# HDSRL/SRB-CBF-NMPC

Hardware: AMD Instinct MI355X
Metric: NMPC solves/sec (whole node) + p99 solve latency, N-agent batch horizon=10 (higher is better)
Workload: dtype f64; 1 GPU; 1024 agents/GPU, horizon 10, 3 static + 8-nearest inter-agent CBF, fp64; agents_per_gpu=1024, agents_total=1024, horizon=10, contacts=2, K_obs=3, K_nbr=8, parallelism=agents sharded x1, n_obs=5120, nbr_rows=1024

## Files before the change

srb-cbf-nmpc_amd/csrc/srb_gram.h:

```cpp
#pragma once
#include <hip/hip_runtime.h>
#include <stdint.h>
#include <type_traits>
#include <utility>
#include "srb_kernel_params.h"
#include "srb_wave.h"

struct TermLayout {
    int N, C, n, nz, E4;
    __device__ __forceinline__ int zr(int v) const { return v < 4 * N ? v : v + E4; }
};

struct ObsFold {
    const double *OJ;
    double *FO;
    int rO, N, K, NOP;
    uint64_t mask;
    int rU, C, n;
};

template <int NZL, bool GRAM, bool RHS>
__device__ __forceinline__ void ul_add(const double *R, const double *W, const double *CF, const ObsFold &F, double *H,
                                       double *g, int nz, int tid0, int step)
{
    constexpr int LDR = NZL + 1, LDH = NZL + 1;
    const int c1 = F.C - 1, np = F.N * c1 * c1, rl = F.rU + 2 * F.N, rs = F.rU + F.n - 1 - 4 * F.N;
    if (GRAM) {
        for (int e = tid0; e <= np; e += step) {
            if (e == np) { H[0] = H[0] + W[rs]; continue; }
            const int j = e / (c1 * c1), rem = e - j * c1 * c1, a = 1 + j * c1 + rem / c1, b = 1 + j * c1 + rem % c1;
            double wv[6], ra[6], rb[6];
#pragma unroll
            for (int u = 0; u < 6; u++) {
                const bool in = u < 2 + F.C;
                const int r = (u < 2) ? F.rU + 2 * j + u : rl + F.C * j + (in ? u - 2 : 0);
                wv[u] = in ? W[r] : 0.0; ra[u] = in ? R[r * LDR + a] : 0.0; rb[u] = in ? R[r * LDR + b] : 0.0;
            }
            const double h0 = H[a * LDH + b];
            __builtin_amdgcn_sched_barrier(0);
            double v = 0.0;
#pragma unroll
            for (int u = 0; u < 6; u++) {
                if (u >= 2 + F.C) break;
                v = fma(wv[u] * ra[u], rb[u], v);
            }
            H[a * LDH + b] = h0 + v;
        }
    }
    if (RHS) {
        for (int a = tid0; a < nz; a += step) {
            if (a == 0) { g[0] += CF[rs]; continue; }
            const int j = (a - 1) / c1;
            double cv[6], ra[6];
#pragma unroll
            for (int u = 0; u < 6; u++) {
                const bool in = u < 2 + F.C;
                const int r = (u < 2) ? F.rU + 2 * j + u : rl + F.C * j + (in ? u - 2 : 0);
                cv[u] = in ? CF[r] : 0.0; ra[u] = in ? R[r * LDR + a] : 0.0;
            }
            const double g0 = g[a];
            __builtin_amdgcn_sched_barrier(0);
            double v = 0.0;
#pragma unroll
            for (int u = 0; u < 6; u++) {
                if (u >= 2 + F.C) break;
                v = fma(cv[u], ra[u], v);
            }
            g[a] = g0 + v;
        }
    }
}

template <int NZL>
struct UlLane {
    double wv[6], ra[6], rb[6], cv[6], sw, sc;
    int q;
    bool he, ge, hs;
    template <bool GRAM, bool RHS>
    __device__ __forceinline__ void load(const double *R, const double *W, const double *CF, const ObsFold &F, int nz, int lane)
    {
        constexpr int LDR = NZL + 1;
        const int li = lane & 15, kq = lane >> 4;
        const int c1 = F.C - 1, rl = F.rU + 2 * F.N, rs = F.rU + F.n - 1 - 4 * F.N;
        const bool col = li >= 1 && li < nz;
        const int j = col ? (li - 1) / c1 : 0, a0 = 1 + j * c1, off = (kq - a0) & 3;
        he = GRAM && col && off < c1;
        ge = RHS && col && kq == 0;
        hs = lane == 0;
        const int a = he ? a0 + off : 1, b = col ? li : 1;
        q = a >> 2;
#pragma unroll
        for (int u = 0; u < 6; u++) {
            const bool in = u < 2 + F.C;
            const int r = (u < 2) ? F.rU + 2 * j + u : rl + F.C * j + (in ? u - 2 : 0);
            if (GRAM) { wv[u] = W[r]; ra[u] = R[r * LDR + a]; }
            rb[u] = R[r * LDR + b];
            if (RHS) cv[u] = CF[r];
        }
        if (GRAM) sw = W[rs];
        if (RHS) sc = CF[rs];
    }
    template <bool GRAM, bool RHS>
    __device__ __forceinline__ void sums(const ObsFold &F, double &vh, double &vg) const
    {
        vh = 0.0; vg = 0.0;
#pragma unroll
        for (int u = 0; u < 6; u++) {
            if (u >= 2 + F.C) break;
            if (GRAM) vh = fma(wv[u] * ra[u], rb[u], vh);
            if (RHS) vg = fma(cv[u], rb[u], vg);
        }
    }
};

template <bool GRAM>
__device__ __forceinline__ void obs_fold(const double *W, const double *CF, const ObsFold &F, int tid, int NTH)
{
    for (int k = tid; k < F.N; k += NTH) {
        double s00 = 0.0, s01 = 0.0, s02 = 0.0, s11 = 0.0, s12 = 0.0, s22 = 0.0, c0 = 0.0, c1 = 0.0, c2 = 0.0;
        for (int j0 = 0; j0 < F.K; j0 += 8) {
            double cfv[8], jxv[8], jyv[8], wv[8];
#pragma unroll
            for (int u = 0; u < 8; u++) {
                const bool in = j0 + u < F.K;
                const int o = k * F.K + (in ? j0 + u : 0);
                cfv[u] = in ? CF[F.rO + o] : 0.0; jxv[u] = in ? F.OJ[2 * o] : 0.0; jyv[u] = in ? F.OJ[2 * o + 1] : 0.0;
                wv[u] = (GRAM && in) ? W[F.rO + o] : 0.0;
            }
#pragma unroll
            for (int u = 0; u < 8; u++) {
                if (j0 + u >= F.K) break;
                const double cf = cfv[u], jx = jxv[u], jy = jyv[u];
                c0 = fma(cf, jx, c0); c1 = fma(cf, jy, c1); c2 -= cf;
                if (GRAM) {
                    const double w = wv[u], wx = w * jx, wy = w * jy;
                    s00 = fma(wx, jx, s00); s01 = fma(wx, jy, s01); s02 -= wx; s11 = fma(wy, jy, s11); s12 -= wy; s22 += w;
                }
            }
        }
        double *f = F.FO + 9 * k;
        if (GRAM) { f[0] = s00; f[1] = s01; f[2] = s02; f[3] = s11; f[4] = s12; f[5] = s22; }
        f[6] = c0; f[7] = c1; f[8] = c2;
    }
}

__device__ __forceinline__ int term_maxcol(int t, int N, int C, int n, int rC, int NE, int rU)
{
    const int c1 = C - 1;
    if (t < rC) return (t / 4 + 1) * c1;
    if (t < rC + NE) return ((t - rC) / 2 + 2) * c1;
    if (t < rU) return 0;
    const int v = 4 * N + (t - rU);
    if (v < 6 * N) return ((v - 4 * N) / 2 + 1) * c1;
    if (v < n - 1) return ((v - 6 * N) / C + 1) * c1;
    return 0;
}

template <int NZM>
__device__ __forceinline__ uint64_t full_batches(int rO, int N, int C, int n, int rC, int NE, int rU, int lane)
// ... 418 lines not shown
            g[tid] = v;
        }
        __syncthreads();
        ul_add<NZL, true, RHS>(R, W, CF, F, H, g, nz, tid, 64 * NW);
    }
}

template <int NZL, int NW>
__device__ __forceinline__ void rhs_only(const double *R, const double *CF, int cnt, const ObsFold &F, int nko, double *g,
                                         int nz, int tid, double *part, uint64_t bmask)
{
    constexpr int NZM = ((NZL + 15) / 16) * 16;
    constexpr int NTC = NZM / 16;
    const int lane = tid & 63, wv = tid >> 6;
    const int li = lane & 15, kq = lane >> 4;
    constexpr bool FOLD = !SRB_OBS_STORED(NZL);
    if (FOLD && nko > 0) {
        obs_fold<false>(nullptr, CF, F, tid, 64 * NW);
        srb_sync<NW>();
    }
    double ps[2][NTC];
    constexpr bool ULF = NZM == 16 && NW == 1;
    UlLane<NZL> ul;
    double ulh = 0.0, ulg = 0.0;
#pragma unroll
    for (int t = 0; t < NTC; t++) { ps[0][t] = 0.0; ps[1][t] = 0.0; }
    auto chunk32 = [&](int t0, auto fullc) {
        constexpr int NB = decltype(fullc)::value ? NTC : 1;
        double a[8][NTC], c[8];
#pragma unroll
        for (int u = 0; u < 8; u++) {
            const int r = t0 + 4 * u + kq;
            c[u] = CF[r];
#pragma unroll
            for (int tc = 0; tc < NB; tc++) a[u][tc] = term_elem<NZL>(R, r, 16 * tc + li);
        }
        __builtin_amdgcn_sched_barrier(0);
#pragma unroll
        for (int u = 0; u < 8; u++)
#pragma unroll
            for (int tc = 0; tc < NB; tc++) ps[u & 1][tc] = fma(c[u], a[u][tc], ps[u & 1][tc]);
    };
    auto schunk16 = [&](int t0, auto fullc) {
        constexpr int NB = decltype(fullc)::value ? NTC : 1;
        double a[4][NTC], c[4];
#pragma unroll
        for (int u = 0; u < 4; u++) {
            const int r = t0 + 4 * u + kq;
            c[u] = CF[r];
#pragma unroll
            for (int tc = 0; tc < NB; tc++) a[u][tc] = term_elem<NZL>(R, r, 16 * tc + li);
        }
        __builtin_amdgcn_sched_barrier(0);
#pragma unroll
        for (int u = 0; u < 4; u++)
#pragma unroll
            for (int tc = 0; tc < NB; tc++) ps[u & 1][tc] = fma(c[u], a[u][tc], ps[u & 1][tc]);
    };
    auto ochunk16 = [&](int t0, auto fullc) {
        constexpr int NB = decltype(fullc)::value ? NTC : 1;
        double a[4][NTC], c[4];
#pragma unroll
        for (int u = 0; u < 4; u++) {
            const int t = t0 + 4 * u + kq, k = t / 3, uu = t - 3 * k;
            c[u] = F.FO[9 * min(k, F.N) + 6 + uu];
#pragma unroll
            for (int tc = 0; tc < NB; tc++) {
                double zx, zy;
                a[u][tc] = obs_term_a<NZL>(R, F, t, 16 * tc + li, zx, zy);
            }
        }
        __builtin_amdgcn_sched_barrier(0);
#pragma unroll
        for (int u = 0; u < 4; u++)
#pragma unroll
            for (int tc = 0; tc < NB; tc++) ps[u & 1][tc] = fma(c[u], a[u][tc], ps[u & 1][tc]);
    };
    auto range = [&](int tb, int te, bool st) {
        int t0 = tb;
#pragma clang loop unroll(disable)
        for (; t0 + 32 <= te; t0 += 32) {
            if (NZM == 16 || st || batch_full(bmask, t0) || batch_full(bmask, t0 + 16))
                chunk32(t0, std::integral_constant<bool, true>{});
            else
                chunk32(t0, std::integral_constant<bool, false>{});
        }
#pragma clang loop unroll(disable)
        for (; t0 < te; t0 += 4) {
            const int r = t0 + kq;
            const double cc = CF[r];
#pragma unroll
            for (int tc = 0; tc < NTC; tc++) ps[0][tc] = fma(cc, term_elem<NZL>(R, r, 16 * tc + li), ps[0][tc]);
        }
    };
    if constexpr (ULF) ul.template load<false, true>(R, nullptr, CF, F, nz, lane);
    {
        constexpr bool ILV = NZM == 32 && NW > 1;
        const int chunk = cnt / NW, tb = wv * chunk;
        if constexpr (ILV) {
#pragma clang loop unroll(disable)
            for (int t0 = 16 * wv; t0 < cnt; t0 += 16 * NW) {
                if (batch_full(bmask, t0)) schunk16(t0, std::integral_constant<bool, true>{});
                else schunk16(t0, std::integral_constant<bool, false>{});
            }
        } else {
            range(tb, tb + chunk, false);
        }
        if (!FOLD && nko > 0) {
            const int och = nko / NW, ob = F.rO + wv * och;
            range(ob, ob + och, true);
        }
        if (FOLD && nko > 0) {
            const int och = F.NOP / NW, ob = ILV ? 16 * wv : wv * och, oe = ILV ? F.NOP : ob + och, os = ILV ? 16 * NW : 16;
#pragma clang loop unroll(disable)
            for (int o0 = ob; o0 < oe; o0 += os) {
                if (NZM == 16 || batch_full(F.mask, o0)) ochunk16(o0, std::integral_constant<bool, true>{});
                else ochunk16(o0, std::integral_constant<bool, false>{});
            }
        }
    }
    if constexpr (ULF) ul.template sums<false, true>(F, ulh, ulg);
    double sv[NTC];
#pragma unroll
    for (int tc = 0; tc < NTC; tc++) sv[tc] = chunk_sum16(ps[0][tc] + ps[1][tc]);
    if constexpr (NW <= 2) {
#pragma unroll
        for (int ph = 0; ph < NW; ph++) {
            if (ph > 0) __syncthreads();
            if (wv == ph) {
#pragma unroll
                for (int tc = 0; tc < NTC; tc++)
                    if (kq == 0 && 16 * tc + li < nz) {
                        if constexpr (ULF) g[li] = ul.ge ? sv[0] + ulg : ul.hs ? sv[0] + ul.sc : sv[0];
                        else g[16 * tc + li] = ph ? g[16 * tc + li] + sv[tc] : sv[tc];
                    }
                if (ph == NW - 1 && !ULF) ul_add<NZL, false, true>(R, nullptr, CF, F, nullptr, g, nz, lane, 64);
            }
        }
    } else {
#pragma unroll
        for (int tc = 0; tc < NTC; tc++)
            if (kq == 0) part[wv * NZM + 16 * tc + li] = sv[tc];
        __syncthreads();
        if (tid < nz) {
            double v = 0.0;
#pragma unroll
            for (int w2 = 0; w2 < NW; w2++) v += part[w2 * NZM + tid];
            g[tid] = v;
        }
        __syncthreads();
        ul_add<NZL, false, true>(R, nullptr, CF, F, nullptr, g, nz, tid, 64 * NW);
    }
}
```

srb-cbf-nmpc_amd/csrc/srb_kernels.hip:

```cpp
#include <hip/hip_runtime.h>
#include <stdint.h>
#include <type_traits>
#include "srb_kernel_params.h"
#include "srb_kernel_decls.h"

#define WAVE 64
#include "srb_wave.h"
#include "srb_gj.h"
#include "srb_solve.h"
#include "srb_gram.h"
#define SYNC() srb_sync<NW>()

#ifdef SRB_STAMPS
#define SRB_NSTAMP 64
__device__ unsigned long long srb_stamp_buf[SRB_NSTAMP];
#define STAMP_DECL unsigned long long st_t0 = 0; int st_off = 0
#define STAMP_BEGIN() do { __builtin_amdgcn_sched_barrier(0); st_t0 = __builtin_amdgcn_s_memtime(); __builtin_amdgcn_sched_barrier(0); } while (0)
#define STAMP_END(slot) do { __builtin_amdgcn_sched_barrier(0); const unsigned long long _t = __builtin_amdgcn_s_memtime(); \
    __builtin_amdgcn_sched_barrier(0); if (threadIdx.x == 0 && stamp_lds) atomicAdd(&stamp_lds[st_off + (slot)], _t - st_t0); st_t0 = _t; } while (0)
#define STAMP_STAGE(s) (st_off = 32 * (s))
#define STAMP_FLUSH(agent) do { SYNC(); if ((agent) == 0 && threadIdx.x < 64) atomicAdd(&srb_stamp_buf[threadIdx.x], stamp_lds[threadIdx.x]); } while (0)
#else
#define STAMP_DECL do {} while (0)
#define STAMP_BEGIN() do {} while (0)
// ... 137 lines not shown
#define SK_KIND(q, t) (TK::compiled ? TK::kind(q, t) : kind_of(q))
#define SK_EQ(t, kd, k) (TK::compiled ? TK::eq(t, kd, k) : (kd) == (k))
#define SK_M(q, t, r) (TK::compiled ? TK::m(q, t, r) : (q).m[r])
#define SK_TWO(t) (!TK::compiled || TK::two(t))
#define SK_ON(t) (TK::compiled && TK::on(t))
#define SK_COM(t) (!TK::compiled || TK::com(t))

template <class TK>
__device__ __forceinline__ double slot_fx(const Slot &q, int t, double x0, double x1, double s_var)
{
    const int k = SK_KIND(q, t);
    const double dx = x0 - q.a0, dy = x1 - q.a1;
    return SK_EQ(t, k, K_OBS) ? -(dx * dx + dy * dy) - s_var : SK_EQ(t, k, K_COP) ? x0 - x1 : x0;
}
template <class TK>
__device__ __forceinline__ double slot_f(const Slot &q, int t, const double *xs, double s_var)
{
    return slot_fx<TK>(q, t, xs[q.i0], xs[q.i1], s_var);
}



__device__ __forceinline__ double zo_sum(const double *zo, int k, int K)
{
    const double *z = zo + k * K;
    double s = 0.0;
    for (int j0 = 0; j0 < K; j0 += 16) {
        double v[16];
#pragma unroll
        for (int u = 0; u < 16; u++) v[u] = (j0 + u < K) ? z[j0 + u] : 0.0;
#pragma unroll
        for (int u = 0; u < 16; u++) s += v[u];
    }
    return s;
}

__device__ __forceinline__ void slot_init(Slot &q, int sl, const SrbKParams &prm, const TermLayout &TL, const double *ref,
                                          int sE, int sV, int sO, int S, int rC, int rO, int K, int TT)
{
    const int N = prm.N, n = prm.n;
    q.kind = K_NONE; q.i0 = q.i1 = 0; q.r = 0; q.h[0] = q.h[1] = 0.0; q.a0 = q.a1 = 0.0; q.rx = 0.0; q.jd = 0.0;
    q.m[0] = q.m[1] = 0.0; q.wr = TT;
    if (sl < SRB_SLOT_END(K_VAR, sE, sV, sO, S)) {
        const int v = sl;
        const bool isX = v < 4 * N, isU = !isX && v < 6 * N, isL = !isX && !isU && v < n - 1;
        q.kind = K_VAR; q.i0 = q.i1 = v; q.r = TL.zr(v);
        q.a0 = isX ? ((v >= 4 * (N - 1)) ? prm.Pw : prm.Qw) : isU ? prm.Rw : isL ? 0.0 : prm.Sw;
        q.a1 = isX ? -q.a0 * ref[v] : 0.0;
        q.h[0] = isL ? 1.0 : prm.box; q.h[1] = isL ? 0.0 : prm.box;
    } else if (sl < SRB_SLOT_END(K_COP, sE, sV, sO, S)) {
        const int e = sl - sE, i = e >> 1, d = e & 1;
        q.kind = K_COP; q.i0 = 4 * i + 2 * d; q.i1 = 4 * N + 2 * (i + 1) + d; q.r = rC + e;
        q.h[0] = q.h[1] = prm.fr;
    } else if (sl < SRB_SLOT_END(K_VEL, sE, sV, sO, S)) {
        const int tt = sl - sV, comp = (tt < N) ? 1 : 3, k = tt % N;
        q.kind = K_VEL; q.i0 = q.i1 = 4 * k + comp; q.r = 4 * k + comp;
        q.h[0] = q.h[1] = prm.vsat;
    } else if (sl < SRB_SLOT_END(K_OBS, sE, sV, sO, S)) {
        const int o = sl - sO, k = o / K;
        q.kind = K_OBS; q.i0 = 4 * k; q.i1 = 4 * k + 2; q.r = rO + o;
    }
#pragma unroll
    for (int r = 0; r < 2; r++) { q.s[r] = q.z[r] = 1.0; q.iz[r] = q.is[r] = 1.0; q.dz[r] = q.ds[r] = q.dsT[r] = q.r3[r] = 0.0; }
}

template <class TK>
__device__ __forceinline__ void slot_stage(Slot &q, int t, int n, bool nl, int TT)
{
    const bool lin = (SK_ISP(q, t, K_VAR) && (SK_ON(t) || q.i0 < n - 1)) || SK_ISP(q, t, K_COP);
    q.m[0] = (lin || (nl && (SK_ISP(q, t, K_VEL) || SK_ISP(q, t, K_OBS)))) ? 1.0 : 0.0;
    q.m[1] = (lin || (nl && SK_ISP(q, t, K_VEL))) ? 1.0 : 0.0;
    q.wr = (SK_ISP(q, t, K_VAR) || SK_ISP(q, t, K_COP) || SK_ISP(q, t, K_OBS)) ? q.r : TT;
}

#define SRB_SLOT_LCK(q, sl) do { \
    LCK((q).wr <= TT, 2); \
    LCK((q).kind == K_NONE || ((q).i0 >= 0 && (q).i0 < n && (q).i1 >= 0 && (q).i1 < n), 3); \
    LCK(!((q).kind == K_VAR || (q).kind == K_COP || (q).kind == K_VEL || ((q).kind == K_OBS && SRB_OBS_STORED(NZL))) || \
        ((q).r >= 0 && (q).r < RROWS), 1); \
    LCK((q).kind != K_OBS || ((sl) - sO >= 0 && (sl) - sO < NK && (q).r - rO == (sl) - sO), 5); \
} while (0)

__device__ __forceinline__ double var_weight(const SrbKParams &prm, int v)
{
    const int N = prm.N;
    return v < 4 * N ? ((v >= 4 * (N - 1)) ? prm.Pw : prm.Qw) : v < 6 * N ? prm.Rw : v < prm.n - 1 ? 0.0 : prm.Sw;
}

template <int NZL, int TS, int NW, class TK>
__device__ __forceinline__ void polish_rows(Slot (&Q)[TS], int nts, const double *xs, double *OJ, double *zo, int n,
                                            int rO, double *R, int nz)
{
    const double s_var = xs[n - 1];
#pragma unroll
    for (int t = 0; t < TS; t++)
        if (t < nts) {
            Slot &q = Q[t];
            q.jd = slot_f<TK>(q, t, xs, s_var);
            if (SK_IS(q, t, K_OBS)) {
                const int o = q.r - rO;
                obs_relin<NZL>(R, OJ, rO, o, q.i0, q.i1, -2.0 * (xs[q.i0] - q.a0), -2.0 * (xs[q.i1] - q.a1));
                zo[o] = q.ds[0] * q.dz[0];
            }
        }
}

__device__ __forceinline__ double lip_eq_res(const SrbKParams &prm, const double *x0, const double *xs, const double *foot,
                                             int N, int C, int tid, int NTH)
{
    double r = 0.0;
#if defined(SRB_DIAG_FLAT_EQRES)
#ifndef SRB_DIAG_BUILD
#error "SRB_DIAG_FLAT_EQRES is a diagnostic-build option"
#endif
    for (int k = tid; k < N; k += NTH) {
        const double *xp = k ? xs + 4 * (k - 1) : x0;
        const double p0 = xp[0], p1 = xp[1], p2 = xp[2], p3 = xp[3];
#else
    const double g0x = x0[0], g1x = x0[1], g2x = x0[2], g3x = x0[3];
    for (int k = tid; k < N; k += NTH) {
        const int kp = k ? k - 1 : 0;
        const double p0 = k ? xs[4 * kp] : g0x, p1 = k ? xs[4 * kp + 1] : g1x;
        const double p2 = k ? xs[4 * kp + 2] : g2x, p3 = k ? xs[4 * kp + 3] : g3x;
#endif
        const double u0 = xs[4 * N + 2 * k], u1 = xs[4 * N + 2 * k + 1];
#pragma unroll
        for (int d = 0; d < 4; d++) {
            const double v = prm.Ad[4 * d] * p0 + prm.Ad[4 * d + 1] * p1 + prm.Ad[4 * d + 2] * p2 +
                             prm.Ad[4 * d + 3] * p3 + prm.Bd[2 * d] * u0 + prm.Bd[2 * d + 1] * u1;
            r = fmax(r, fabs(xs[4 * k + d] - v));
        }
        double g0 = 0.0, g1 = 0.0, sl = 0.0;
#pragma unroll
        for (int j = 0; j < 4; j++)
            if (j < C) {
                const double lam = xs[6 * N + C * k + j];
                g0 = fma(foot[(2 * k) * C + j], lam, g0); g1 = fma(foot[(2 * k + 1) * C + j], lam, g1); sl += lam;
            }
        r = fmax(r, fmax(fabs(u0 - g0), fmax(fabs(u1 - g1), fabs(sl - 1.0))));
    }
    return r;
}

template <int NZL, int TS, int NW, int NZE, class TK>
__device__ __forceinline__ double polish_stationary(Slot (&Q)[TS], int nts, const SrbKParams &prm, const double *xs,
                                                  const double *ref, double *CF, double *R, double *OJ, double *zo, int rO,
                                                  int cnt, const ObsFold &OF, int nko, double *vg, double *vy, double *vr,
                                                  double *vd, const double (&Mi)[NZL], const double *H0, int nz, int tid,
                                                  double *part, uint64_t bmask, double *red, int N, int n, int TT, int srow)
{
    SYNC();
    polish_rows<NZL, TS, NW, TK>(Q, nts, xs, OJ, zo, n, rO, R, nz);
    SYNC();
#pragma unroll
    for (int t = 0; t < TS; t++)
        if (t < nts) {
            const Slot &q = Q[t];
            const double zj = SK_TWO(t) ? q.ds[0] * q.dz[0] - q.ds[1] * q.dz[1] : q.ds[0] * q.dz[0];
            const int kd = SK_KIND(q, t);
            if (SK_EQ(t, kd, K_VAR)) {
                const int v = q.i0;
                const double a0 = var_weight(prm, v), gf = fma(a0, xs[v], (v < 4 * N) ? -a0 * ref[v] : 0.0);
                CF[q.wr] = gf + zj;
            } else if (SK_EQ(t, kd, K_COP) || SK_EQ(t, kd, K_OBS)) {
                CF[q.wr] = zj;
            }
        }
    if (NW > 1) SYNC();
#pragma unroll
    for (int t = 0; t < TS; t++)
        if (t < nts && SK_IS(Q[t], t, K_VEL))
            __hip_atomic_fetch_add(&CF[Q[t].r], Q[t].ds[0] * Q[t].dz[0] - Q[t].ds[1] * Q[t].dz[1], __ATOMIC_RELAXED,
                                   __HIP_MEMORY_SCOPE_WORKGROUP);
    SYNC();
    rhs_only<NZL, NW>(R, CF, cnt, OF, nko, vg, nz, tid, part, bmask);
    SYNC();
    double dxs[NZL];
    la_solve<NZL, NW, NZE>(Mi, H0, H0, 0.0, vg, vy, vr, vd, dxs, nz, tid & 63);
    double dm = 0.0;
#pragma unroll
    for (int j = 0; j < NZL; j++) dm = fmax(dm, fabs(dxs[j]));
    constexpr int LDR = NZL + 1;
    double zmin = 1e300, zmax = 1.0;
#pragma unroll
    for (int t = 0; t < TS; t++)
        if (t < nts && (Q[t].ds[0] != 0.0 || (SK_TWO(t) && Q[t].ds[1] != 0.0))) {
            const Slot &q = Q[t];
            const double jd = -((!SRB_OBS_STORED(NZL) && SK_IS(q, t, K_OBS))
                ? fma(OJ[2 * (q.r - rO)], row_dot<NZL, NZE>(R + q.i0 * LDR, dxs),
                      fma(OJ[2 * (q.r - rO) + 1], row_dot<NZL, NZE>(R + q.i1 * LDR, dxs), -row_dot<NZL, NZE>(R + srow * LDR, dxs)))
                : row_dot<NZL, NZE>(R + q.r * LDR, dxs));
#pragma unroll
            for (int r = 0; r < 2; r++)
                if ((SK_TWO(t) || r == 0) && q.ds[r] != 0.0) {
                    const double zn = fma(prm.polish_rho, q.r3[r] + (r ? -jd : jd), q.dz[r]);
                    zmin = fmin(zmin, zn); zmax = fmax(zmax, fabs(zn));
                }
        }
    double rv[2] = {-zmin, zmax};
    wred_x<2, 3u, NW>(rv, red + 5 * 8 * NW, tid);
    return (-rv[0] >= -(prm.polish_rho * SRB_POLISH_PTOL + 1e-9 * rv[1])) ? dm : 1e300;
}

#define SRB_AGENT_LAYOUT \
    constexpr int NZM = ((NZL + 15) / 16) * 16; \
    constexpr int LDR = NZL + 1, LDH = NZL + 1; \
    constexpr int NTH = 64 * NW; \
    constexpr int NZE = (NC > 0 && CC > 0) ? NC * (CC - 1) + 1 : NZL;    \
     \
    constexpr bool GVEC = SRB_GRAM_FORM != SRB_GRAM_MFMA && srb_shape_compiled(NC, CC, KC) && NW == 1 && NZL <= 12 && \
                          SRB_OBS_STORED(NZL) && CC > 1 && NZE <= NZL; \
    using GSH = GramShape<GVEC ? NC : 0, GVEC ? CC : 0, GVEC ? KC : 0>; \
    const int tid = threadIdx.x, lane = tid & 63, wv = tid >> 6; \
     \
    const int N = NC > 0 ? NC : prm.N, C = CC > 0 ? CC : prm.C, K = KC > 0 ? KC : prm.K_obs + prm.K_nbr; \
    const int n = (NC > 0 && CC > 0) ? (6 + CC) * NC + 1 : prm.n, nz = (NC > 0 && CC > 0) ? NC * (CC - 1) + 1 : prm.nz; \
    const int NK = N * K, NE = 2 * (N - 1); \
    const int n4 = rnd4(n), NK4 = rnd4(NK), UL4 = rnd4(n - 4 * N); \
    const int E4 = (4 * N + NE + 16 * NW - 1) / (16 * NW) * (16 * NW) - 4 * N;    \
     \
     \
    const int rC = 4 * N, rU = rC + E4, rO = (rU + UL4 + 16 * NW - 1) / (16 * NW) * (16 * NW); \
    const int NKP = (NK + 16 * NW - 1) / (16 * NW) * (16 * NW), TT = rO + NKP; \
    const TermLayout TL{N, C, n, nz, E4}; \
    const uint64_t bmask = full_batches<NZM>(rO, N, C, n, rC, NE, rU, lane);    \
    const int NOP = (3 * N + 16 * NW - 1) / (16 * NW) * (16 * NW);    \
    const int sE = n, sV = n + NE, sO = sV + 2 * N, S = sO + NK; \
    const double tol = prm.tol, th = tol / sqrt(3.0); \
    STAMP_DECL; \
     \
    double *p = lds; \
    double *R = p; p += (SRB_OBS_STORED(NZL) ? TT : rO) * LDR;    \
    double *W = p; p += TT + 1;                    \
    double *CF = p; p += TT + 1;                   \
    double *OJ = p; p += SRB_OBS_STORED(NZL) ? 0 : 2 * NKP;        \
    double *FO = p; p += SRB_OBS_STORED(NZL) ? 0 : 9 * (N + 1);    \
    const ObsFold OF{OJ, FO, rO, N, K, NOP, full_obs_batches<NZM>(N, C, NOP, lane), rU, C, n}; \
    double *H0 = p; p += NZL * LDH;                \
    double *ZZ = p; p += NZL * LDH;                \
    double *vg = p; p += NZM; double *vy = p; p += NZM; double *vr = p; p += NZM; double *vd = p; p += NZM; \
    double *xs = p; p += n4; \
    double *xb = p; p += n4;                       \
    double *dxv = xb; \
    double *xsv = p; p += n4;                      \
    double *xprev = p; p += n4;                    \
    double *ref = p; p += 4 * N; \
    double *foot = p; p += 2 * C * N; \
    double *obs = SRB_OBS_IN_ZZ(NZL, NK) ? ZZ : p; p += SRB_OBS_IN_ZZ(NZL, NK) ? 0 : 2 * NK + 2;    \
    double *eps = p; p += K + 1; \
    double *zo = p; p += NK4;                      \
    int *sel = (int *)p; p += (K + 1); \
    double *red = p; p += (NW > 1) ? 8 * SRB_RED_SITES * NW : 0;    \
    double *part = p; p += (NW > 2) ? NW * ((NZM == 16) ? 1 : 3) * 256 + NW * NZM : 0;    \
    float *zpl = (float *)p; p += SRB_FUSED_POLISH_OK(NZL) ? rnd4(S) : 0;    \
    const int RROWS = SRB_OBS_STORED(NZL) ? TT : rO;    \
    LCK_INIT(); \
    LCK((int)(p - lds) <= srb_lds_doubles(prm, NZL, NW), 0); \
    LCK(rU <= RROWS && (!SRB_OBS_STORED(NZL) || rO + NKP <= TT), 4); \
    (void)RROWS; \
    do {} while (0)

#define SRB_AGENT_SETUP \
    const double *x0 = x0g + 4 * (size_t)agent; \
    for (int i = tid; i < 4 * N; i += NTH) ref[i] = refg[(size_t)agent * 4 * N + i]; \
    for (int i = tid; i < 2 * C * N; i += NTH) foot[i] = footg[(size_t)agent * 2 * C * N + i]; \
    if (prm.use_nlp && tid < K) sel[tid] = sel_g[(size_t)agent * K + tid]; \
    for (int i = tid; i < (int)(xs - R) + 2 * n4; i += NTH) R[i] = 0.0; \
    for (int i = tid; i < NK4; i += NTH) zo[i] = 0.0; \
    SYNC(); \
    STAMP_END(23);                  \
    if (prm.use_nlp) { SRB_AGENT_OBSTACLES; } \
    STAMP_END(24);                  \
     \
    if (tid == 0) { \
        double X[4] = {x0[0], x0[1], x0[2], x0[3]}; \
        for (int k = 0; k < N; k++) { \
            const double u0 = foot[(k * 2 + 0) * C + C - 1], u1 = foot[(k * 2 + 1) * C + C - 1]; \
            double Xn[4]; \
            for (int d = 0; d < 4; d++) \
                Xn[d] = prm.Ad[d * 4] * X[0] + prm.Ad[d * 4 + 1] * X[1] + prm.Ad[d * 4 + 2] * X[2] + prm.Ad[d * 4 + 3] * X[3] + \
                        prm.Bd[d * 2] * u0 + prm.Bd[d * 2 + 1] * u1; \
            for (int d = 0; d < 4; d++) { X[d] = Xn[d]; xb[4 * k + d] = Xn[d]; } \
            xb[4 * N + 2 * k] = u0; xb[4 * N + 2 * k + 1] = u1; \
            for (int j = 0; j < C; j++) xb[6 * N + C * k + j] = (j == C - 1) ? 1.0 : 0.0; \
        } \
        xb[n - 1] = 0.0; \
    } \
    for (int cg = tid; cg < nz - 1; cg += NTH) {    \
        const int j = cg / (C - 1), t = cg % (C - 1), col = cg + 1; \
        double lam[4]; \
        const int is_null = lambda_basis(foot + j * 2 * C, C, t, lam); \
        double g0 = 0.0, g1 = 0.0; \
        if (!is_null) \
            _Pragma("unroll") for (int i = 0; i < 4; i++) \
                if (i < C) { g0 += foot[(j * 2 + 0) * C + i] * lam[i]; g1 += foot[(j * 2 + 1) * C + i] * lam[i]; } \
        _Pragma("unroll") for (int i = 0; i < 4; i++) if (i < C) R[TL.zr(6 * N + C * j + i) * LDR + col] = lam[i]; \
        R[TL.zr(4 * N + 2 * j) * LDR + col] = g0; \
        R[TL.zr(4 * N + 2 * j + 1) * LDR + col] = g1; \
        double v[4]; \
        for (int d = 0; d < 4; d++) v[d] = prm.Bd[d * 2] * g0 + prm.Bd[d * 2 + 1] * g1; \
        for (int k = j; k < N; k++) { \
            for (int d = 0; d < 4; d++) R[(4 * k + d) * LDR + col] = v[d]; \
            double tt[4]; \
            for (int d = 0; d < 4; d++) tt[d] = prm.Ad[d * 4] * v[0] + prm.Ad[d * 4 + 1] * v[1] + prm.Ad[d * 4 + 2] * v[2] + prm.Ad[d * 4 + 3] * v[3]; \
            for (int d = 0; d < 4; d++) v[d] = tt[d]; \
        } \
    } \
    if (tid == 0) R[TL.zr(n - 1) * LDR] = 1.0; \
    SYNC(); \
    STAMP_END(25);                  \
     \
    if (tid < NE) { \
        const int i = tid >> 1, d = tid & 1, pp = 4 * i + 2 * d, uu = 4 * N + 2 * (i + 1) + d; \
        for (int a = 0; a < NZL; a++) Rt[tid * LDR + a] = R[pp * LDR + a] - R[TL.zr(uu) * LDR + a]; \
    } \
    for (int v = tid; v < n; v += NTH) xs[v] = xb[v]; \
    do {} while (0)

#define SRB_AGENT_OBSTACLES \
     \
    { \
        double ox_[TS], oy_[TS]; \
        _Pragma("unroll") for (int t = 0; t < TS; t++) { \
            const int e = tid + NTH * t; \
            ox_[t] = oy_[t] = 0.0; \
            if (e < NK) { \
                const int k = e / K, j = e - k * K; \
                const bool st = j < prm.K_obs; \
                const int bi = sel[j]; \
                const double tt = st ? 0.0 : prm.Ts * (k + 1); \
                const size_t bj = (bi >= 0) ? bi : 0; \
                if (nbr_plan) {    \
                     \
                    const double *srcp = st ? obstacles + 2 * bj : nbr_plan + 2 * (bj * (size_t)N + k); \
                    ox_[t] = (bi >= 0) ? srcp[0] : x0[0] + 1000.0; \
                    oy_[t] = (bi >= 0) ? srcp[1] : x0[2]; \
                } else { \
                    const double *srcp = st ? obstacles + 2 * bj : nbr_state + 4 * bj; \
                     \
                    ox_[t] = (bi >= 0) ? srcp[0] + (st ? 0.0 : srcp[2] * tt) : x0[0] + 1000.0; \
                    oy_[t] = (bi >= 0) ? srcp[1] + (st ? 0.0 : srcp[3] * tt) : x0[2]; \
                } \
                if (MV && obs_vel) {    \
                     \
                     \
                     \
                    _Pragma("clang fp contract(off)") \
                    if (st && bi >= 0) { \
                        const double tk = prm.Ts * (k + 1); \
                        ox_[t] = obstacles[2 * bj] + obs_vel[2 * bj] * tk; \
                        oy_[t] = obstacles[2 * bj + 1] + obs_vel[2 * bj + 1] * tk; \
                    } \
                } \
            } \
        } \
        _Pragma("unroll") for (int t = 0; t < TS; t++) { \
            const int e = tid + NTH * t; \
            if (e < NK) { obs[2 * e] = ox_[t]; obs[2 * e + 1] = oy_[t]; } \
        } \
        if (tid < K) eps[tid] = (tid < prm.K_obs) ? prm.eps_obs : prm.eps_nbr; \
         \
         \
         \
        if (MV && obs_eps) { if (tid < prm.K_obs && sel[tid] >= 0) eps[tid] = obs_eps[sel[tid]]; } \
         \
// ... 521 lines not shown
```

srb-cbf-nmpc_amd/csrc/srb_stage_body.h:

```cpp
        const double tolS = (!nl && prm.use_nlp && prm.qp_warm_tol > 0.0) ? prm.qp_warm_tol : tol, thS = tolS / sqrt(3.0);
        STAMP_STAGE(stage);
        const int nts = ((nl ? S : sV) + NTH - 1) / NTH;
        const int mrows = nl ? (4 * (N - 1) + 12 * N + 2 * C * N + NK + 4 * N) : (4 * (N - 1) + 12 * N + 2 * C * N);
        const int cnt = rU, nko = nl ? NKP : 0;
        STAMP_BEGIN();
#pragma unroll
        for (int t = 0; t < TS; t++) {
            Slot &q = Q[t];
            const bool lin = (SK_ISP(q, t, K_VAR) && (SK_ON(t) || q.i0 < n - 1)) || SK_ISP(q, t, K_COP);
            q.m[0] = (lin || (nl && (SK_ISP(q, t, K_VEL) || SK_ISP(q, t, K_OBS)))) ? 1.0 : 0.0;
            q.m[1] = (lin || (nl && SK_ISP(q, t, K_VEL))) ? 1.0 : 0.0;
            q.wr = (SK_ISP(q, t, K_VAR) || SK_ISP(q, t, K_COP) || SK_ISP(q, t, K_OBS)) ? q.r : TT;
        }
        if (!nl) {
#pragma unroll
            for (int t = 0; t < TS; t++)
                if (SK_TWO(t) && t < nts) {
                    Slot &q = Q[t];
                    const double f = slot_f<TK>(q, t, xs, 0.0);
                    const double w0 = SK_M(q, t, 0) * (q.h[0] - f), w1 = SK_M(q, t, 1) * (q.h[1] + f);
                    const bool var = SK_ISP(q, t, K_VAR);
                    const double wgt = (var ? q.a0 : 0.0) + SK_M(q, t, 0) + SK_M(q, t, 1);
                    const double cfv = (var ? -q.a1 - q.a0 * f : 0.0) + (w0 - w1);
                    if (SK_ISP(q, t, K_VAR) || SK_ISP(q, t, K_COP)) { W[q.r] = wgt; CF[q.r] = cfv; }
// ... 92 lines not shown
#pragma unroll
            for (int t = 0; t < TS; t++)
                if (t < nts) {
                    Slot &q = Q[t];
                    const double f = q.jd;
                    q.s[0] = (SK_M(q, t, 0) != 0.0) ? q.h[0] - f + ssh : 1.0;
                    if (SK_TWO(t)) q.s[1] = (SK_M(q, t, 1) != 0.0) ? q.h[1] + f + ssh : 1.0;
                    q.z[0] = SRB_NLP_Z0 * rcp_d(fmax(q.s[0], 1.0));
                    if (SK_TWO(t)) q.z[1] = SRB_NLP_Z0 * rcp_d(fmax(q.s[1], 1.0));
                    if (SK_ISP(q, t, K_OBS)) {
                        const int o = q.r - rO;
                        obs_relin<NZL>(R, OJ, rO, o, q.i0, q.i1, -2.0 * (xs[q.i0] - q.a0), -2.0 * (xs[q.i1] - q.a1));
                    }
                    const double jz = SK_TWO(t) ? SK_M(q, t, 0) * q.z[0] - SK_M(q, t, 1) * q.z[1] : q.m[0] * q.z[0];
                    if (SK_ISP(q, t, K_VAR)) { W[q.r] = 1.0; CF[q.r] = fma(q.a0, f, q.a1) + jz; }
                    else if (SK_ISP(q, t, K_COP)) { W[q.r] = 0.0; CF[q.r] = jz; }
                    else if (SK_ISP(q, t, K_OBS)) { W[q.r] = 0.0; CF[q.r] = q.z[0]; }
                }
            if (NW > 1) SYNC();
#pragma unroll
            for (int t = 0; t < TS; t++)
                if (t < nts && SK_ISP(Q[t], t, K_VEL))
                    __hip_atomic_fetch_add(&CF[Q[t].r], Q[t].m[0] * Q[t].z[0] - Q[t].m[1] * Q[t].z[1], __ATOMIC_RELAXED,
                                           __HIP_MEMORY_SCOPE_WORKGROUP);
            SYNC();
            if constexpr (GVEC) gram_rhs_vec<NZL, true, GSH, SRB_GRAM_FORM>(R, W, CF, OF, nko, ZZ, vg, nz, lane);
            else gram_rhs<NZL, true, NW>(R, W, CF, cnt, OF, nko, ZZ, vg, nz, tid, part, bmask);
            SYNC();
            gj_load<NZL, NZE>(Mi, ZZ, ZZ, 0.0, nz, lane);
            gj_factor<NZL, NZE>(Mi, nz, lane, 0);
            la_solve<NZL, NW, NZE>(Mi, ZZ, ZZ, 0.0, vg, vy, vr, vd, dxi, nz, lane);
#pragma unroll
            for (int t = 0; t < TS; t++)
                if (t < nts) {
                    Slot &q = Q[t];
                    q.rx = (SK_ISP(q, t, K_VAR)) ? -row_dot<NZL, NZE>(R + q.r * LDR, dxi) : 0.0;
                }
            SYNC();
            STAMP_END(2);
        }

        const int maxit = nl ? prm.nlp_maxit : prm.qp_maxit;
        double sigma = 100.0;
        const double sigma_d = 0.0;
        int flag = 2, it = 0;
        const double inv_m = 1.0 / (double)mrows;
        double dxl = 1e300;
        int npassed = 0;
        bool saved = false, restore = false;
        bool prov = false;
        double best_rx = 1e300;
        auto export_zpol = [&]() {
            const bool to_lds = SRB_FUSED_POLISH_OK(NZL) && prm.polish_fused;
            __attribute__((address_space(1))) float *zg = (__attribute__((address_space(1))) float *)(zpol_g + (size_t)agent * zstride);
            __attribute__((address_space(3))) float *zl = (__attribute__((address_space(3))) float *)zpl;
#pragma unroll
            for (int t = 0; t < TS; t++)
                if (t < nts && tid + NTH * t < S)
#pragma unroll
                    for (int r = 0; r < 2; r++) {
                        const float v = SK_M(Q[t], t, r) == 0.0 ? 0.0f
                            : (float)(Q[t].s[r] * SRB_POLISH_KAPPA < Q[t].z[r] ? Q[t].z[r] : -fmin(Q[t].z[r] / Q[t].s[r], SRB_POLISH_OMCAP));
                        if (to_lds) zl[2 * (tid + NTH * t) + r] = v;
                        else zg[2 * (tid + NTH * t) + r] = v;
                    }
        };
        for (int v = tid; v < n; v += NTH) xprev[v] = xs[v];
        double hsc[TS] = {};
        for (int iter = 0; iter < maxit; iter++) {
            STAMP_BEGIN();
            const double s_var = xs[n - 1];
            double nrx = 0.0, nrz = 0.0, sz = 0.0, gm = 1.0, zmx = 0.0;
            double fv[TS];
            double xa[TS], xc[TS];
#pragma unroll
            for (int t = 0; t < TS; t++) {
                xa[t] = xc[t] = 0.0;
                if (t < nts) { xa[t] = xs[Q[t].i0]; xc[t] = xs[Q[t].i1]; }
            }
#pragma unroll
            for (int t = 0; t < TS; t++) {
                fv[t] = 0.0;
                if (t < nts) {
                    Slot &q = Q[t];
                    const double f = slot_fx<TK>(q, t, xa[t], xc[t], s_var);
                    fv[t] = f;
                    if (SK_IS(q, t, K_VAR)) {
                        nrx = fma(q.rx, q.rx, nrx);
                        gm = fmax(gm, fabs(fma(q.a0, f, q.a1)));
                    }
                    const double m0 = SK_M(q, t, 0), m1 = SK_M(q, t, 1);
                    const double rz0 = q.h[0] - q.s[0] - f;
                    if (SK_TWO(t)) {
                        const double rz1 = q.h[1] - q.s[1] + f;
                        nrz = fma(m0 * rz0, rz0, fma(m1 * rz1, rz1, nrz));
                        sz = fma(m0 * q.s[0], q.z[0], fma(m1 * q.s[1], q.z[1], sz));
                        zmx = fmax(zmx, fmax(m0 * q.z[0], m1 * q.z[1]));
                    } else {
                        nrz = fma(m0 * rz0, rz0, nrz);
                        sz = fma(m0 * q.s[0], q.z[0], sz);
                        zmx = fmax(zmx, m0 * q.z[0]);
                    }
                    if constexpr (!LEAN)
#pragma unroll
                        for (int r = 0; r < 2; r++)
                            if (SK_TWO(t) || r == 0) { q.iz[r] = rcp_d(q.z[r]); q.is[r] = rcp_d(q.s[r]); }
                    if (nl && SK_IS(q, t, K_OBS)) {
                        const int o = q.r - rO;
                        obs_relin<NZL>(R, OJ, rO, o, q.i0, q.i1, -2.0 * (xa[t] - q.a0), -2.0 * (xc[t] - q.a1));
                        zo[o] = q.z[0];
                    }
                }
            }
            STAMP_END(18);
            double dxm;
            {
                double rv[6] = {nrx, nrz, sz, gm, dxl, zmx};
                wred_x<6, 56u, NW>(rv, red + 2 * 8 * NW, tid);
                nrx = sqrt(rv[0]); nrz = sqrt(rv[1]); sz = rv[2]; gm = rv[3]; dxm = rv[4]; zmx = rv[5];
            }
            const double mu = sz * inv_m;
            const bool f32 = KF && mu > prm.kkt32_mu;
            (void)f32;
            STAMP_END(3);
            if (!isfinite(nrx) || !isfinite(nrz) || !isfinite(sz) || !(zmx <= SRB_Z_DIV)) {
                flag = 3;
                if (!isfinite(nrx) || !isfinite(nrz) || !isfinite(sz)) {
                    SYNC();
                    for (int v = tid; v < n; v += NTH) xs[v] = xprev[v];
                    SYNC();
                }
                break;
            }
            const double thx = nl ? SRB_NLP_EXITF * th * gm : thS;
            const double mtol = nl ? SRB_NLP_EXITF * tol : tolS;
            NLPDBG(iter, 0, nrx); NLPDBG(iter, 1, thx); NLPDBG(iter, 2, nrz); NLPDBG(iter, 3, sz * inv_m);
            const bool pass = nrx < thx && nrz < thS && sz * inv_m < mtol;
            if (pass && (!nl || dxm < SRB_NLP_DXTOL)) {
                prov = nl && !(nrx < th * gm && sz * inv_m < tol);
                flag = 0; break;
            }
            const bool near = nl && nrz < th && sz * inv_m < mtol && nrx < 100.0 * thx;
            if (nl && saved && !near) { restore = true; flag = 4; break; }
            if (near && nrx / gm <= best_rx) {
                best_rx = nrx / gm;
                for (int v = tid; v < n; v += NTH) xsv[v] = xs[v];
                if (zpol_g || prm.polish_fused) export_zpol();
                saved = true;
            }
            if (near && ++npassed >= SRB_NLP_NEARWAIT) { flag = 4; break; }
            bool acc = false;
            const bool pc = nl || (sigma > sigma_d);
            double delta = 0.0;
            auto set_rhs = [&](int pass) {
                const double smu = (pass == 0) ? 0.0 : (pc ? sigma * mu : sigma_d * mu);
                const bool corr = pass == 1 && pc;
                double cfs[TS];
#pragma unroll
                for (int t = 0; t < TS; t++) {
                    cfs[t] = 0.0;
                    if (t < nts) {
                        Slot &q = Q[t];
                        const double f = fv[t];
                        double cf = (SK_IS(q, t, K_VAR)) ? q.rx : 0.0;
#pragma unroll
                        for (int r = 0; r < 2; r++)
                            if (SK_TWO(t) || r == 0) {
                                double dsT = -q.s[r] * q.z[r];
                                if constexpr (SPLIT) {
                                    if (corr) dsT = fma(-q.ds[r], q.dz[r], dsT);
                                    dsT = add_plain(dsT, smu);
                                } else {
                                    if (corr) dsT -= q.ds[r] * q.dz[r];
                                    dsT += smu;
                                }
                                const double rz = r ? (q.h[1] - q.s[1] + f) : (q.h[0] - q.s[0] - f);
                                const double r3 = fma(-dsT, IZ(q, r), rz);
                                if constexpr (!LEAN) { q.dsT[r] = dsT; q.r3[r] = r3; }
                                cf = fma((r ? -SK_M(q, t, 1) : SK_M(q, t, 0)) * q.z[r] * IS(q, r), r3, cf);
                            }
                        cfs[t] = cf;
                        CF[q.wr] = cf;
                    }
                }
                if (NW > 1) SYNC();
                if (nl)
#pragma unroll
                    for (int t = 0; t < TS; t++)
                        if (t < nts && SK_IS(Q[t], t, K_VEL))
                            __hip_atomic_fetch_add(&CF[Q[t].r], cfs[t], __ATOMIC_RELAXED, __HIP_MEMORY_SCOPE_WORKGROUP);
            };
            if (pc) {
                SYNC();
#pragma unroll
                for (int t = 0; t < TS; t++)
                    if (t < nts) {
                        Slot &q = Q[t];
                        const double om = SK_TWO(t) ? fma(SK_M(q, t, 0) * q.z[0], IS(q, 0), SK_M(q, t, 1) * q.z[1] * IS(q, 1))
                                                     : q.m[0] * q.z[0] * IS(q, 0);
                        double hs = 0.0;
                        if (nl && SK_COM(t) && SK_IS(q, t, K_VAR) && q.i0 < 4 * N && !(q.i0 & 1)) {
                            const int k = q.i0 >> 2;
                            if constexpr (TK::compiled) {
                                if (iter == 0) hsc[t] = zo_sum(zo, k, K);
                                hs = hsc[t];
                            } else {
                                hs = zo_sum(zo, k, K);
                            }
                            hs *= -2.0;
                        }
                        W[q.wr] = om + ((SK_IS(q, t, K_VAR)) ? q.a0 + hs : 0.0);
                    }
                if (NW > 1) SYNC();
                if (nl)
#pragma unroll
                    for (int t = 0; t < TS; t++)
                        if (t < nts && SK_IS(Q[t], t, K_VEL))
                            __hip_atomic_fetch_add(&W[Q[t].r], Q[t].z[0] * IS(Q[t], 0) + Q[t].z[1] * IS(Q[t], 1), __ATOMIC_RELAXED,
                                                   __HIP_MEMORY_SCOPE_WORKGROUP);
                STAMP_END(16);
                set_rhs(0);
                SYNC();
                STAMP_END(17);
                if constexpr (GVEC) gram_rhs_vec<NZL, true, GSH, SRB_GRAM_FORM>(R, W, CF, OF, nko, H0, vg, nz, lane);
                else gram_rhs<NZL, true, NW>(R, W, CF, cnt, OF, nko, H0, vg, nz, tid, part, bmask);
                SYNC();
                STAMP_END(4);
                int ok = 0;
                const int ntries = nl ? 14 : 1;
                for (int tries = 0; tries < ntries; tries++) {
                    LCK(nl || delta == 0.0, 7);
                    gj_load<NZL, NZE>(Mi, H0, ZZ, delta, nz, lane);
                    int cf = (KF && f32) ? gj_invert_f32<NZL>(Mi, mrow<NZL>(lane), !nl) : gj_factor<NZL, NZE>(Mi, nz, lane, !nl);
#ifdef SRB_DIAG_FORCE_SHIFT
#ifndef SRB_DIAG_BUILD
#error "SRB_DIAG_FORCE_SHIFT is a diagnostic-build option"
#endif
                    if (nl && tries == 0) cf = 1;
#endif
                    if (cf == 0) { ok = 1; break; }
                    if (tries + 1 == ntries) break;
                    if (delta == 0.0) {
                        const double dm = (lane < nz) ? H0[lane * LDH + lane] : 1.0;
                        delta = 1e-10 * fmax(1.0, wmax(dm));
                    } else {
                        delta *= 10.0;
                    }
                }
                STAMP_END(5);
                if (!ok) { flag = 1; break; }
                if (near && delta != 0.0) { flag = 4; break; }
            }

            double ap = 1.0, ad = 1.0;
#pragma clang loop unroll(disable)
            for (int pass = (pc ? 0 : 1); pass < 2; pass++) {
                if (pass == 1 || !pc) {
                    set_rhs(pass);
                    SYNC();
                    STAMP_END(6 + 4 * pass);
                    rhs_only<NZL, NW>(R, CF, cnt, OF, nko, vg, nz, tid, part, bmask);
                    SYNC();
                    STAMP_END(7 + 4 * pass);
                }
                la_solve<NZL, NW, NZE, KF>(Mi, H0, ZZ, delta, vg, vy, vr, vd, dxi, nz, lane, (KF && f32) ? prm.kkt32_ref : SRB_REFINE);
                STAMP_END(8 + 4 * pass);
                double mxs = 0.0, mxz = 0.0;
                if constexpr (!SRB_OBS_STORED(NZL)) {
                    for (int v = tid; v < n; v += NTH) dxv[v] = row_dot<NZL, NZE>(R + TL.zr(v) * LDR, dxi);
                    SYNC();
                }
                double rw[SRB_OBS_STORED(NZL) ? 2 : 1][NZE];
                if constexpr (SRB_OBS_STORED(NZL))
                    if (0 < nts) row_load<NZE>(R + Q[0].r * LDR, rw[0]);
#pragma unroll
                for (int t = 0; t < TS; t++)
                    if (t < nts) {
                        Slot &q = Q[t];
                        const int kd = SK_KIND(q, t);
                        if constexpr (SRB_OBS_STORED(NZL)) {
                            LCK(q.r >= 0 && q.r < RROWS, 1);
                            if (t + 1 < TS && t + 1 < nts) row_load<NZE>(R + Q[(t + 1) % TS].r * LDR, rw[(t + 1) & 1]);
                            __builtin_amdgcn_sched_barrier(0);
                            q.jd = row_sum<NZL, NZE>(rw[t & 1], dxi);
                        } else if (SK_EQ(t, kd, K_OBS)) {
                            const int o = q.r - rO;
                            q.jd = nl ? fma(OJ[2 * o], dxv[q.i0], fma(OJ[2 * o + 1], dxv[q.i1], -dxv[n - 1])) : 0.0;
                        } else {
                            q.jd = SK_EQ(t, kd, K_COP) ? dxv[q.i0] - dxv[q.i1] : dxv[q.i0];
                        }
#pragma unroll
                        for (int r = 0; r < 2; r++)
                        if (SK_TWO(t) || r == 0) {
                            const double izr = IZ(q, r), isr = IS(q, r);
                            double dsT, r3;
                            if constexpr (LEAN) {
                                dsT = -q.s[r] * q.z[r];
                                if (pass == 1 && pc) dsT -= q.ds[r] * q.dz[r];
                                dsT += (pass == 0) ? 0.0 : (pc ? sigma * mu : sigma_d * mu);
                                const double rz = r ? (q.h[1] - q.s[1] + fv[t]) : (q.h[0] - q.s[0] - fv[t]);
                                r3 = fma(-dsT, izr, rz);
                            } else {
                                dsT = q.dsT[r]; r3 = q.r3[r];
                            }
                            q.dz[r] = SK_M(q, t, r) * q.z[r] * isr * fma(r ? -1.0 : 1.0, q.jd, -r3);
                            q.ds[r] = SK_M(q, t, r) * fma(-q.s[r], q.dz[r], dsT) * izr;
                            mxs = fmax(mxs, -q.ds[r] * isr); mxz = fmax(mxz, -q.dz[r] * izr);
                        }
                    }
                STAMP_END(21 + pass);
                {
                    double rv[2] = {mxs, mxz};
                    wred_x<2, 3u, NW>(rv, red + (3 + 2 * pass) * 8 * NW, tid);
                    mxs = rv[0]; mxz = rv[1];
                }
                ap = (mxs > 0.0) ? 1.0 / mxs : 1.0;
                ad = (mxz > 0.0) ? 1.0 / mxz : 1.0;
                STAMP_END(9 + 4 * pass);
                if (pass == 0) {
                    double num = 0.0;
#pragma unroll
                    for (int t = 0; t < TS; t++)
                        if (t < nts) {
                            const Slot &q = Q[t];
                            num = fma(SK_M(q, t, 0) * fma(ap, q.ds[0], q.s[0]), fma(ad, q.dz[0], q.z[0]), num);
                            if (SK_TWO(t)) num = fma(SK_M(q, t, 1) * fma(ap, q.ds[1], q.s[1]), fma(ad, q.dz[1], q.z[1]), num);
                        }
                    {
                        double rv[1] = {num};
                        wred_x<1, 0u, NW>(rv, red + 4 * 8 * NW, tid);
                        num = rv[0];
                    }
                    const double rho = num / sz, mr = rho < 1.0 ? rho : 1.0;
                    sigma = mr * mr * mr; if (sigma < sigma_d) sigma = sigma_d;
                    continue;
                }
                if (near && (ap < SRB_NLP_BLOCKED || ad < SRB_NLP_BLOCKED)) { acc = true; break; }
                ap = (0.99 * ap < 1.0) ? 0.99 * ap : 1.0;
                ad = (0.99 * ad < 1.0) ? 0.99 * ad : 1.0;
                dxl = 0.0;
                NLPDBG(iter, 4, ap); NLPDBG(iter, 5, ad); NLPDBG(iter, 6, delta); NLPDBG(iter, 7, sigma);
                double hso[TS];
#pragma unroll
                for (int t = 0; t < TS; t++) {
                    hso[t] = 0.0;
                    if (t < nts) {
                        Slot &q = Q[t];
                        if (nl && SK_COM(t) && SK_IS(q, t, K_VAR) && q.i0 < 4 * N && !(q.i0 & 1)) {
                            const int k = q.i0 >> 2;
                            if constexpr (TK::compiled) hso[t] = hsc[t];
                            else hso[t] = zo_sum(zo, k, K);
                        }
#pragma unroll
                        for (int r = 0; r < 2; r++)
                            if (SK_TWO(t) || r == 0) { q.s[r] = fma(ap, q.ds[r], q.s[r]); q.z[r] = fma(ad, q.dz[r], q.z[r]); }
                    }
                }
                SYNC();
                STAMP_END(19);
#pragma unroll
                for (int t = 0; t < TS; t++)
                    if (t < nts) {
                        Slot &q = Q[t];
                        if (nl && SK_IS(q, t, K_OBS)) zo[q.r - rO] = q.z[0];
                        if (SK_IS(q, t, K_VAR)) {
                            dxl = fmax(dxl, fabs(ap * q.jd));
                            q.rx = (1.0 - ad) * q.rx + ((ad - ap) * q.a0) * q.jd;
                            if (nl) q.rx = fma(ad * (delta - 2.0 * hso[t]), q.jd, q.rx);
                            xprev[q.i0] = fv[t];
                            xs[q.i0] = fma(ap, q.jd, fv[t]);
                        }
                    }
                SYNC();
                STAMP_END(20);
                if (nl)
#pragma unroll
                    for (int t = 0; t < TS; t++)
                        if (t < nts) {
                            Slot &q = Q[t];
                            if (SK_COM(t) && SK_IS(q, t, K_VAR) && q.i0 < 4 * N && !(q.i0 & 1)) {
                                const int k = q.i0 >> 2;
                                double hs_new = 0.0;
                                hs_new = zo_sum(zo, k, K);
                                if constexpr (TK::compiled) hsc[t] = hs_new;
                                q.rx = fma(2.0 * ap * hs_new, q.jd, q.rx);
                            }
                        }
                STAMP_END(14);
            }
            if (acc) { flag = 4; break; }
            it++;
        }
        if (flag == 0 && prov) flag = 4;
        if (nl && saved && !prov && (restore || flag == 2 || flag == 4)) {
            for (int v = tid; v < n; v += NTH) xs[v] = xsv[v];
            flag = 4;
        } else if ((zpol_g || prm.polish_fused) && nl) {
            export_zpol();
        }
        if (stage == 0) { qp_flag = (flag == 0 && tolS > tol) ? 4 : flag; qp_it = it; } else { nlp_flag = flag; nlp_it = it; }
```

Baseline: 5.556 million solves/s.

## Compute KKT right-hand side directly from per-thread slot coefficients in registers

```diff
diff --git a/srb-cbf-nmpc_amd/csrc/srb_gram.h b/srb-cbf-nmpc_amd/csrc/srb_gram.h
--- a/srb-cbf-nmpc_amd/csrc/srb_gram.h
+++ b/srb-cbf-nmpc_amd/csrc/srb_gram.h
@@ -5,6 +5,7 @@
 #include <utility>
 #include "srb_kernel_params.h"
 #include "srb_wave.h"
+#include "srb_solve.h"
 
 struct TermLayout {
     int N, C, n, nz, E4;
@@ -729,3 +730,46 @@
         ul_add<NZL, false, true>(R, nullptr, CF, F, nullptr, g, nz, tid, 64 * NW);
     }
 }
+
+#ifndef SRB_RHS_SLOTS
+#define SRB_RHS_SLOTS 1
+#endif
+#ifndef SRB_RHS_SLOTS_QP
+#define SRB_RHS_SLOTS_QP 0
+#endif
+constexpr bool srb_rhs_slots(bool compiled, int NW, int NZL, int NZE)
+{
+    return SRB_RHS_SLOTS && compiled && NW == 1 && NZL <= 12 && SRB_OBS_STORED(NZL) && NZE > 1 && NZE <= NZL;
+}
+
+template <int NZL, int NZE, int TS>
+__device__ __forceinline__ void rhs_slots(const double *R, const double (&cfs)[TS], const int (&rows)[TS], int nts, double *g,
+                                          int nz, int lane)
+{
+    static_assert(NZE <= 12 && NZE <= NZL, "rhs_slots: one column block of at most 12 columns");
+    constexpr int LDR = NZL + 1;
+    const int li = lane & 15, kq = lane >> 4;
+    double acc[12];
+#pragma unroll
+    for (int j = 0; j < 12; j++) acc[j] = 0.0;
+    double rw[2][NZE];
+    if (0 < nts) row_load<NZE>(R + rows[0] * LDR, rw[0]);
+#pragma unroll
+    for (int t = 0; t < TS; t++)
+        if (t < nts) {
+            if (t + 1 < TS && t + 1 < nts) row_load<NZE>(R + rows[(t + 1) % TS] * LDR, rw[(t + 1) & 1]);
+            __builtin_amdgcn_sched_barrier(0);
+#pragma unroll
+            for (int j = 0; j < NZE; j++) acc[j] = fma(cfs[t], rw[t & 1][j], acc[j]);
+        }
+    d4 d = gram_scatter(acc);
+#define SRB_RS_STAGE(CTRL) { const double t0_ = dpp_d<CTRL>(d[0]), t1_ = dpp_d<CTRL>(d[1]), t2_ = dpp_d<CTRL>(d[2]); \
+                             d[0] += t0_; d[1] += t1_; d[2] += t2_; }
+    SRB_RS_STAGE(0xB1) SRB_RS_STAGE(0x4E) SRB_RS_STAGE(0x141) SRB_RS_STAGE(0x140)
+#undef SRB_RS_STAGE
+    if (li == 0) {
+#pragma unroll
+        for (int q = 0; q < 3; q++)
+            if (kq + 4 * q < nz) g[kq + 4 * q] = d[q];
+    }
+}
diff --git a/srb-cbf-nmpc_amd/csrc/srb_kernels.hip b/srb-cbf-nmpc_amd/csrc/srb_kernels.hip
--- a/srb-cbf-nmpc_amd/csrc/srb_kernels.hip
+++ b/srb-cbf-nmpc_amd/csrc/srb_kernels.hip
@@ -313,6 +313,27 @@
     SYNC();
     polish_rows<NZL, TS, NW, TK>(Q, nts, xs, OJ, zo, n, rO, R, nz);
     SYNC();
+    if constexpr (srb_rhs_slots(TK::compiled, NW, NZL, NZE)) {
+        double cfs[TS];
+        int rr[TS];
+#pragma unroll
+        for (int t = 0; t < TS; t++) {
+            const Slot &q = Q[t];
+            cfs[t] = 0.0; rr[t] = q.r;
+            if (t < nts) {
+                const double zj = SK_TWO(t) ? q.ds[0] * q.dz[0] - q.ds[1] * q.dz[1] : q.ds[0] * q.dz[0];
+                const int kd = SK_KIND(q, t);
+                if (SK_EQ(t, kd, K_VAR)) {
+                    const int v = q.i0;
+                    const double a0 = var_weight(prm, v), gf = fma(a0, xs[v], (v < 4 * N) ? -a0 * ref[v] : 0.0);
+                    cfs[t] = gf + zj;
+                } else if (SK_EQ(t, kd, K_COP) || SK_EQ(t, kd, K_OBS) || SK_EQ(t, kd, K_VEL)) {
+                    cfs[t] = zj;
+                }
+            }
+        }
+        rhs_slots<NZL, NZE, TS>(R, cfs, rr, nts, vg, nz, tid & 63);
+    } else {
 #pragma unroll
     for (int t = 0; t < TS; t++)
         if (t < nts) {
@@ -335,6 +356,7 @@
                                    __HIP_MEMORY_SCOPE_WORKGROUP);
     SYNC();
     rhs_only<NZL, NW>(R, CF, cnt, OF, nko, vg, nz, tid, part, bmask);
+    }
     SYNC();
     double dxs[NZL];
     la_solve<NZL, NW, NZE>(Mi, H0, H0, 0.0, vg, vy, vr, vd, dxs, nz, tid & 63);
@@ -372,6 +394,8 @@
     constexpr bool GVEC = SRB_GRAM_FORM != SRB_GRAM_MFMA && srb_shape_compiled(NC, CC, KC) && NW == 1 && NZL <= 12 && \
                           SRB_OBS_STORED(NZL) && CC > 1 && NZE <= NZL; \
     using GSH = GramShape<GVEC ? NC : 0, GVEC ? CC : 0, GVEC ? KC : 0>; \
+     \
+    constexpr bool RSL = srb_rhs_slots(srb_shape_compiled(NC, CC, KC), NW, NZL, NZE); \
     const int tid = threadIdx.x, lane = tid & 63, wv = tid >> 6; \
      \
     const int N = NC > 0 ? NC : prm.N, C = CC > 0 ? CC : prm.C, K = KC > 0 ? KC : prm.K_obs + prm.K_nbr; \
diff --git a/srb-cbf-nmpc_amd/csrc/srb_stage_body.h b/srb-cbf-nmpc_amd/csrc/srb_stage_body.h
--- a/srb-cbf-nmpc_amd/csrc/srb_stage_body.h
+++ b/srb-cbf-nmpc_amd/csrc/srb_stage_body.h
@@ -268,6 +268,7 @@
             bool acc = false;
             const bool pc = nl || (sigma > sigma_d);
             double delta = 0.0;
+            constexpr bool RSLS = RSL && (nl || SRB_RHS_SLOTS_QP);
             auto set_rhs = [&](int pass) {
                 const double smu = (pass == 0) ? 0.0 : (pc ? sigma * mu : sigma_d * mu);
                 const bool corr = pass == 1 && pc;
@@ -296,9 +297,11 @@
                                 cf = fma((r ? -SK_M(q, t, 1) : SK_M(q, t, 0)) * q.z[r] * IS(q, r), r3, cf);
                             }
                         cfs[t] = cf;
+                        if constexpr (RSLS) { if (pass != 0) { q.jd = cf; continue; } }
                         CF[q.wr] = cf;
                     }
                 }
+                if constexpr (RSLS) { if (pass != 0) return; }
                 if (NW > 1) SYNC();
                 if (nl)
 #pragma unroll
@@ -372,10 +375,20 @@
 #pragma clang loop unroll(disable)
             for (int pass = (pc ? 0 : 1); pass < 2; pass++) {
                 if (pass == 1 || !pc) {
-                    set_rhs(pass);
-                    SYNC();
-                    STAMP_END(6 + 4 * pass);
-                    rhs_only<NZL, NW>(R, CF, cnt, OF, nko, vg, nz, tid, part, bmask);
+                    if constexpr (RSLS) {
+                        set_rhs(1);
+                        STAMP_END(6 + 4 * pass);
+                        double cfr[TS];
+                        int rr[TS];
+#pragma unroll
+                        for (int t = 0; t < TS; t++) { cfr[t] = Q[t].jd; rr[t] = Q[t].r; }
+                        rhs_slots<NZL, NZE, TS>(R, cfr, rr, nts, vg, nz, lane);
+                    } else {
+                        set_rhs(pass);
+                        SYNC();
+                        STAMP_END(6 + 4 * pass);
+                        rhs_only<NZL, NW>(R, CF, cnt, OF, nko, vg, nz, tid, part, bmask);
+                    }
                     SYNC();
                     STAMP_END(7 + 4 * pass);
                 }
```

Result: faster. 5.716 million solves/s, median of 6 (+2.9%).
